# zgbkdlm/fbs

Hardware: AMD Instinct MI355X
Metric: particle-steps/sec (N x T per Gibbs sweep) (higher is better)
Workload: dtype f32; 1 GPU; 2-D Gaussian bridge toy (BASELINE config 2): N=65536 particles, T=500 steps, ts=linspace(0,2), analytic score, gibbs_kernel eb=True ef=False marg_y=False, conditional killing resampling; one step = one Gibbs sweep of a batch of 4 chain(s) (reference driver default nchains=4, vmapped); nparticles=65536, nsteps=500, nchains=4, du=1, dv=1, parallelism=1 GPU(s) x 4 independent chain(s) each, no collective

## Files before the change

### fbs_amd/csrc/fbsmi_lg.hip

```cpp
#include <hip/hip_runtime.h>

#include <array>
#include <cmath>
#include <cstdlib>
#include <map>
#include <mutex>
#include <new>
#include <string>
#include <utility>
#include <vector>

#include "../../include/fbsmi.h"
#include "fbsmi_device.h"
#include "fbsmi_em_path.h"
#include "fbsmi_host.h"

namespace fbsmi {

constexpr int kMaxNbSweep = 1024;
constexpr int kNumProfKernels = 3;

struct LgDev {
    int C;
    int Ctot, c0;
// ... 1379 lines not shown
    constexpr bool kPairNoise = DMAX <= 4;
    constexpr bool kEarlyRow = DMAX <= 2;
    const LgDev d = chain_view(dd, blockIdx.y);
    __shared__ TreeLds L;
    __shared__ float part[2][4 * HALVES];
    __shared__ int Jsh;
    __shared__ float lastsh;
    __shared__ float xish[kPairNoise ? DMAX : 1][NP];
    const int N = d.N, tid = threadIdx.x & (kBlock - 1), half = threadIdx.x / kBlock, lane = threadIdx.x & 63;
    const bool upper = half >= HP;
    const int pr = (int)threadIdx.x - (upper ? NP : 0);
    const int mL = blockIdx.x * NP + pr;
    const int m = upper ? mL + (N >> 1) : mL;
    const int tileb = m / kBlock;
    const uint32_t* kt = d.keytab + 8 * s;
    const uint32_t a0 = kt[0], a1 = kt[1], b0 = kt[2], b1 = kt[3], t0 = kt[6], t1 = kt[7];
    const int i_ref = d.bs[s], j_ref = d.bs[s + 1];
    const float* __restrict__ up = (s & 1) ? d.u1 : d.u0;
    float* __restrict__ un = (s & 1) ? d.u0 : d.u1;
    const float w_max = d.scal[1];
    const float inv_n = 1.0f / (float)N;
    TreeEntry te{};
    if (half == 0) te = tree_entry_loads(d, i_ref);
    float uref[DMAX];
#pragma unroll
    for (int r = 0; r < DMAX; ++r) uref[r] = r < d.du ? up[(size_t)r * N + i_ref] : 0.0f;
    const StepTables<DMAX> t = step_tables<DMAX>(d, s);
    const float* v_prev = d.vs + (size_t)s * d.dv;
    const float* v = d.vs + (size_t)(s + 1) * d.dv;
    const float* ustar = d.us_star + (size_t)(s + 1) * d.du;
    const float u3 = __uint_as_float(kt[4]);
    float xi[DMAX];
#pragma unroll
    for (int r = 0; r < DMAX; ++r) xi[r] = 0.0f;
    if (!kPairNoise) {
#pragma unroll
        for (int r = 0; r < DMAX; ++r)
            if (r < d.du) xi[r] = normal_at(t0, t1, (uint64_t)N * d.du, (uint64_t)m * d.du + r);
    } else if (upper) {
#pragma unroll
        for (int r = 0; r < DMAX; ++r) {
            if (r < d.du) {
                uint32_t lo_, hi_;
                random_bits_pair(t0, t1, (uint64_t)N * d.du, (uint64_t)mL * d.du + r, lo_, hi_);
                xish[r][pr] = normal_from_bits(lo_);
                xi[r] = normal_from_bits(hi_);
            }
        }
    }
    float last;
    int J;
    if (half == 0) {
        float rootW;
        J = tree_build(d, te, L, i_ref, u3, w_max, inv_n, last, rootW);
        if (tid == 0) {
            Jsh = J;
            lastsh = last;
        }
    } else {
#pragma unroll
        for (int k = 0; k < kTreeBuildBarriers; ++k) __syncthreads();
    }
    __syncthreads();
    J = Jsh;
    last = lastsh;
    int shift = (j_ref - J) % N;
    if (shift < 0) shift += N;
    int src = m - shift;
    if (src < 0) src += N;
    const float ws = d.w[src];
    float u[DMAX];
#pragma unroll
    for (int r = 0; r < DMAX; ++r) u[r] = r < d.du ? up[(size_t)r * N + src] : 0.0f;
    if (kPairNoise && !upper) {
#pragma unroll
        for (int r = 0; r < DMAX; ++r)
            if (r < d.du) xi[r] = xish[r][pr];
    }
    const float u1 = uniform_at(a0, a1, (uint64_t)N, (uint64_t)src);
    const float u2 = uniform_at(b0, b1, (uint64_t)N, (uint64_t)src);
    const float q = last * (1.0f - u2);
    float P = 0.0f, E = last;
    int tile, h, red = 0;
    tree_search_lds(L, d.nb, q, P, E, tile, h);
    const bool killed = u1 * w_max >= ws;
    float ucand[DMAX];
    if (killed) {
        const TreeRound rd = tree_round_load(d, tile, h);
        const int lo = tree_round_walk(rd, tile, h, q, P, E);
        const float4 w4 = *reinterpret_cast<const float4*>(d.w + lo);
        float4 ug[DMAX];
        float ue[DMAX];
        if (kEarlyRow) {
            const int en = lo + 4 < N ? lo + 4 : N - 1;
#pragma unroll
            for (int r = 0; r < DMAX; ++r) {
                ug[r] = r < d.du ? *reinterpret_cast<const float4*>(up + (size_t)r * N + lo) : make_float4(0.f, 0.f, 0.f, 0.f);
                ue[r] = r < d.du ? up[(size_t)r * N + en] : 0.0f;
            }
        }
        red = tree_leaves_walk(w4, lo, q, P, E);
        if (kEarlyRow) {
            const int k = red - lo;
#pragma unroll
            for (int r = 0; r < DMAX; ++r) {
                const float lo2 = (k & 1) ? ug[r].y : ug[r].x, hi2 = (k & 1) ? ug[r].w : ug[r].z;
                ucand[r] = k >= 4 ? ue[r] : ((k & 2) ? hi2 : lo2);
            }
        }
    }
    const bool pinned = m == j_ref;
    const int a = pinned ? i_ref : (killed ? red : src);
    if (killed && !pinned) {
#pragma unroll
        for (int r = 0; r < DMAX; ++r)
            if (r < d.du) u[r] = kEarlyRow ? ucand[r] : up[(size_t)r * N + a];
    }
    if (pinned) {
#pragma unroll
        for (int r = 0; r < DMAX; ++r) u[r] = uref[r];
    }
    if (d.As) d.As[(size_t)s * N + m] = a;
#pragma unroll
    for (int r = 0; r < DMAX; ++r) {
        if (r < d.du) {
            const float dr = drift_row<DMAX>(t, r, u, v_prev);
            float x = (u[r] + dr * t.dt) + t.sd * xi[r];
            if (pinned) x = ustar[r];
            un[(size_t)r * N + m] = x;
            if (d.uss) d.uss[((size_t)(s + 1) * N + m) * d.du + r] = x;
        }
    }
    const float l = lg_loglik<DMAX>(t, u, v, v_prev);
    d.lw[m] = l;
    float mx, sx;
    {
        const int wv = (threadIdx.x >> 6) & 3, h4 = half * 4;
        const float mw = wave_max(l);
        if (lane == 0) part[0][h4 + wv] = mw;
        __syncthreads();
        mx = fmaxf(fmaxf(part[0][h4], part[0][h4 + 1]), fmaxf(part[0][h4 + 2], part[0][h4 + 3]));
        TreePath pth;
        const float sw_ = wave_upsweep(fbsmi_expf(l - finite_or_zero_f(mx)), pth);
        if (lane == 0) part[1][h4 + wv] = sw_;
        __syncthreads();
        sx = (part[1][h4] + part[1][h4 + 1]) + (part[1][h4 + 2] + part[1][h4 + 3]);
    }
    if (tid == 0) {
        d.bmax[tileb] = mx;
        d.bsumexp[tileb] = sx;
    }
}

template <int DMAX>
__global__ void __launch_bounds__(kBlock) k_lg_prop2t(LgDev dd, int s) {
    const LgDev d = chain_view(dd, blockIdx.y);
    __shared__ TreeLds L;
    __shared__ float xch2[2][8];
    const int N = d.N, half = N >> 1, tid = threadIdx.x;
    const uint32_t* kt = d.keytab + 8 * s;
    const uint32_t a0 = kt[0], a1 = kt[1], b0 = kt[2], b1 = kt[3], t0 = kt[6], t1 = kt[7];
    const int i_ref = d.bs[s], j_ref = d.bs[s + 1];
    const int mA = blockIdx.x * kBlock + tid;
    const int m[2] = {mA, mA + half};
    const float* __restrict__ up = (s & 1) ? d.u1 : d.u0;
    float* __restrict__ un = (s & 1) ? d.u0 : d.u1;
    const float w_max = d.scal[1];
    const float inv_n = 1.0f / (float)N;
    const TreeEntry te = tree_entry_loads(d, i_ref);
    float uref[DMAX];
#pragma unroll
    for (int r = 0; r < DMAX; ++r) uref[r] = r < d.du ? up[(size_t)r * N + i_ref] : 0.0f;
    const StepTables<DMAX> t = step_tables<DMAX>(d, s);
    const float* v_prev = d.vs + (size_t)s * d.dv;
    const float* v = d.vs + (size_t)(s + 1) * d.dv;
    const float* ustar = d.us_star + (size_t)(s + 1) * d.du;
    const float u3 = __uint_as_float(kt[4]);
    float xi[2][DMAX];
#pragma unroll
    for (int r = 0; r < DMAX; ++r) {
        xi[0][r] = 0.0f;
        xi[1][r] = 0.0f;
        if (r < d.du) {
            uint32_t lo_, hi_;
            random_bits_pair(t0, t1, (uint64_t)N * d.du, (uint64_t)mA * d.du + r, lo_, hi_);
            xi[0][r] = normal_from_bits(lo_);
            xi[1][r] = normal_from_bits(hi_);
        }
    }
    float last;
    float rootW_unused;
    const int J = tree_build(d, te, L, i_ref, u3, w_max, inv_n, last, rootW_unused);
    int shift = (j_ref - J) % N;
    if (shift < 0) shift += N;
    int src[2];
    src[0] = mA - shift;
    if (src[0] < 0) src[0] += N;
    const bool a_low = src[0] < half;
    src[1] = a_low ? src[0] + half : src[0] - half;
    const int pbase = a_low ? src[0] : src[1];
    float ws[2], u[2][DMAX];
#pragma unroll
    for (int h2 = 0; h2 < 2; ++h2) {
        ws[h2] = d.w[src[h2]];
#pragma unroll
        for (int r = 0; r < DMAX; ++r) u[h2][r] = r < d.du ? up[(size_t)r * N + src[h2]] : 0.0f;
    }
    uint32_t k_lo, k_hi, r_lo, r_hi;
    random_bits_pair(a0, a1, (uint64_t)N, (uint64_t)pbase, k_lo, k_hi);
    random_bits_pair(b0, b1, (uint64_t)N, (uint64_t)pbase, r_lo, r_hi);
    const float u1[2] = {fbsmi_bits_to_unit(a_low ? k_lo : k_hi), fbsmi_bits_to_unit(a_low ? k_hi : k_lo)};
    const float u2[2] = {fbsmi_bits_to_unit(a_low ? r_lo : r_hi), fbsmi_bits_to_unit(a_low ? r_hi : r_lo)};
    const float qK[2] = {last * (1.0f - u2[0]), last * (1.0f - u2[1])};
    float P[2] = {0.0f, 0.0f}, E[2] = {last, last};
    int tile[2], h[2], hi[2] = {0, 0};
    {
        auto walk2x2 = [&](const float2* hp0, const float2* hp1, int& h0, int& h1) {
            const float2 a0 = hp0[h0], a1 = hp1[h1];
            const float4 c0 = *reinterpret_cast<const float4*>(hp0 + 2 * h0), c1 = *reinterpret_cast<const float4*>(hp1 + 2 * h1);
            const bool g0 = tree_walk(a0, qK[0], P[0], E[0]), g1 = tree_walk(a1, qK[1], P[1], E[1]);
            const bool k0 = tree_walk(g0 ? make_float2(c0.x, c0.y) : make_float2(c0.z, c0.w), qK[0], P[0], E[0]);
            const bool k1 = tree_walk(g1 ? make_float2(c1.x, c1.y) : make_float2(c1.z, c1.w), qK[1], P[1], E[1]);
            h0 = 4 * h0 + (g0 ? 0 : 2) + (k0 ? 0 : 1);
            h1 = 4 * h1 + (g1 ? 0 : 2) + (k1 ? 0 : 1);
        };
        auto walk1x2 = [&](const float2* hp0, const float2* hp1, int& h0, int& h1) {
            const float2 n0 = hp0[h0], n1 = hp1[h1];
            h0 = 2 * h0 + (tree_walk(n0, qK[0], P[0], E[0]) ? 0 : 1);
            h1 = 2 * h1 + (tree_walk(n1, qK[1], P[1], E[1]) ? 0 : 1);
        };
        const int nb = d.nb;
        int h0 = kBlock / nb, h1 = h0, lv = 31 - __builtin_clz(nb);
        for (; lv >= 2; lv -= 2) walk2x2(L.topW, L.topW, h0, h1);
        if (lv) walk1x2(L.topW, L.topW, h0, h1);
        tile[0] = h0 - kBlock;
        tile[1] = h1 - kBlock;
        const float2 *m0 = L.midW + tile[0] * kMidN, *m1 = L.midW + tile[1] * kMidN;
        h0 = h1 = 1;
        static_assert(kMidLv == 3 || kMidLv == 4, "walk of the tile levels kept in LDS");
        walk2x2(m0, m1, h0, h1);
        if (kMidLv == 4) walk2x2(m0, m1, h0, h1);
        else walk1x2(m0, m1, h0, h1);
        h[0] = h0;
        h[1] = h1;
    }
    const bool killed[2] = {u1[0] * w_max >= ws[0], u1[1] * w_max >= ws[1]};
    {
        TreeRound rd0{}, rd1{};
        if (killed[0]) rd0 = tree_round_load(d, tile[0], h[0]);
        if (killed[1]) rd1 = tree_round_load(d, tile[1], h[1]);
        int lo0 = 0, lo1 = 0;
        float4 w40 = make_float4(0.f, 0.f, 0.f, 0.f), w41 = w40;
        if (killed[0]) {
            lo0 = tree_round_walk(rd0, tile[0], h[0], qK[0], P[0], E[0]);
            w40 = *reinterpret_cast<const float4*>(d.w + lo0);
        }
        if (killed[1]) {
            lo1 = tree_round_walk(rd1, tile[1], h[1], qK[1], P[1], E[1]);
            w41 = *reinterpret_cast<const float4*>(d.w + lo1);
        }
        if (killed[0]) hi[0] = tree_leaves_walk(w40, lo0, qK[0], P[0], E[0]);
        if (killed[1]) hi[1] = tree_leaves_walk(w41, lo1, qK[1], P[1], E[1]);
    }
    float lnew[2];
#pragma unroll
    for (int h2 = 0; h2 < 2; ++h2) {
        const bool pinned = m[h2] == j_ref;
        const int a = pinned ? i_ref : (killed[h2] ? hi[h2] : src[h2]);
        if (killed[h2] && !pinned) {
#pragma unroll
            for (int r = 0; r < DMAX; ++r)
                if (r < d.du) u[h2][r] = up[(size_t)r * N + a];
        }
        if (pinned) {
#pragma unroll
            for (int r = 0; r < DMAX; ++r) u[h2][r] = uref[r];
        }
        if (d.As) d.As[(size_t)s * N + m[h2]] = a;
#pragma unroll
        for (int r = 0; r < DMAX; ++r) {
            if (r < d.du) {
                const float dr = drift_row<DMAX>(t, r, u[h2], v_prev);
                float x = (u[h2][r] + dr * t.dt) + t.sd * xi[h2][r];
                if (pinned) x = ustar[r];
                un[(size_t)r * N + m[h2]] = x;
                if (d.uss) d.uss[((size_t)(s + 1) * N + m[h2]) * d.du + r] = x;
            }
        }
        lnew[h2] = lg_loglik<DMAX>(t, u[h2], v, v_prev);
        d.lw[m[h2]] = lnew[h2];
    }
    float mxA, sxA, mxB, sxB;
    block_lse_partial2(lnew[0], lnew[1], xch2[0], xch2[1], mxA, sxA, mxB, sxB);
    if (tid == 0) {
        const int tb = blockIdx.x + (d.nb >> 1);
        d.bmax[blockIdx.x] = mxA;
        d.bsumexp[blockIdx.x] = sxA;
        d.bmax[tb] = mxB;
        d.bsumexp[tb] = sxB;
    }
}

template <int DMAX>
__global__ void __launch_bounds__(kBlock) k_lg_prop2(LgDev dd, int s) {
    const LgDev d = chain_view(dd, blockIdx.y);
    __shared__ float xch[2][8];
// ... 1582 lines not shown
    const float diff = prop_ell - old_ell;
    const float log_acc = (diff < 0.0f || diff != diff) ? diff : 0.0f;
    const float z = uniform_at(p.pk[4 * c + 2], p.pk[4 * c + 3], 1, 0);
    const bool acc = fbsmi_logf(z) < log_acc;
    __syncthreads();
    float* samples = (float*)p.out[0];
    float* uT = p.uT + (size_t)c * p.du;
    const float* new_uT = p.usT + ((size_t)c * p.N + p.which_u) * p.du;
    for (int r = threadIdx.x; r < p.du; r += kBlock) {
        const float x = acc ? new_uT[r] : uT[r];
        uT[r] = x;
        if (samples) samples[((size_t)it * p.C + c) * p.du + r] = x;
    }
    if (acc) {
        const size_t nys = ((size_t)p.T + 1) * p.dv;
        float* ys = p.ys + (size_t)c * nys;
        const float* prop = p.prop_ys + (size_t)c * nys;
        for (size_t e = threadIdx.x; e < nys; e += kBlock) ys[e] = prop[e];
    }
    if (threadIdx.x == 0) {
        if (acc) p.log_ell[c] = prop_ell;
        const size_t o = (size_t)it * p.C + c;
        if (p.out[1]) ((float*)p.out[1])[o] = fbsmi_expf(log_acc);
        if (p.out[2]) ((uint8_t*)p.out[2])[o] = acc ? 1 : 0;
        if (p.out[3]) ((float*)p.out[3])[o] = prop_ell;
        if (p.out[4]) ((float*)p.out[4])[o] = old_ell;
    }
}

constexpr int kFsBlockMax = 128;

__global__ void __launch_bounds__(kFsBlockMax) k_fs_front(PmDev p) {
    const int b = blockIdx.y;
    __shared__ uint32_t sk[2];
    __shared__ float syT[kFsBlockMax];
    if (threadIdx.x == 0) {
        const uint32_t k0 = p.ikeys[2 * b], k1 = p.ikeys[2 * b + 1];
        uint32_t f0, f1;
        split_at(k0, k1, 3, 0, sk[0], sk[1]);
        split_at(k0, k1, 3, 2, f0, f1);
        p.fkeys[2 * b] = f0;
        p.fkeys[2 * b + 1] = f1;
        split_at(f0, f1, 2, 0, p.pk[4 * b], p.pk[4 * b + 1]);
    }
    __syncthreads();
    const int T = p.T, dv = p.dv;
    const bool live = (int)threadIdx.x < dv;
    const int j = live ? (int)threadIdx.x : dv - 1;
    const uint32_t s0 = sk[0], s1 = sk[1];
    const uint64_t n = (uint64_t)T * dv;
    float* vs = p.vs + (size_t)b * ((size_t)T + 1) * dv;
    float r = p.y0[j];
    if (live) vs[(size_t)T * dv + j] = r;
    for (int k0 = 0; k0 < T; k0 += kPmChunk) {
        float f[kPmChunk], sq[kPmChunk], z[kPmChunk];
#pragma unroll
        for (int i = 0; i < kPmChunk; ++i) {
            const int k = k0 + i < T ? k0 + i : T - 1;
            f[i] = p.F[k];
            sq[i] = p.sqQ[k];
            z[i] = normal_at(s0, s1, n, (uint64_t)k * dv + j);
        }
#pragma unroll
        for (int i = 0; i < kPmChunk; ++i) {
            if (k0 + i < T) {
                r = f[i] * r + sq[i] * z[i];
                if (live) vs[(size_t)(T - 1 - k0 - i) * dv + j] = r;
            }
        }
    }
    if (live) syT[j] = r;
    __syncthreads();
    for (int u = threadIdx.x; u < p.du; u += blockDim.x) {
        double s = 0.0;
        for (int cc = 0; cc < dv; ++cc) s = s + p.gain[(size_t)u * dv + cc] * ((double)syT[cc] - p.m_v[cc]);
        p.mcond[(size_t)b * p.du + u] = (float)(p.m_u[u] + s);
    }
}

__global__ void __launch_bounds__(kFsBlockMax) k_fs_tail(PmDev p) {
    const int b = blockIdx.y;
    const float* row0 = p.usT + (size_t)b * p.N * p.du;
    for (int r = threadIdx.x; r < p.du; r += blockDim.x) p.uT[(size_t)b * p.du + r] = row0[r];
    if (threadIdx.x == 0) p.log_ell[b] = p.ell[b];
}

}

using namespace fbsmi;

__global__ void k_xcc_probe(int* out) {
    if (threadIdx.x == 0) {
        uint32_t id;
        asm volatile("s_getreg_b32 %0, hwreg(HW_REG_XCC_ID)" : "=s"(id));
        out[blockIdx.x] = (int)(id & 15);
    }
}

static bool xcd_round_robin_holds() {
    static const int ok = [] {
        if (const char* e = getenv("FBSMI_PIN_CHECK"))
            if (atoi(e) == 0) return 1;
        constexpr int kProbeBlocks = 64;
        int* dev = nullptr;
        int host[kProbeBlocks];
        if (hipMalloc(&dev, sizeof(host)) != hipSuccess) return 0;
        bool good = hipMemset(dev, 0xff, sizeof(host)) == hipSuccess;
        if (good) {
            k_xcc_probe<<<kProbeBlocks, 64, 0, nullptr>>>(dev);
            good = hipMemcpy(host, dev, sizeof(host), hipMemcpyDeviceToHost) == hipSuccess;
        }
        (void)hipFree(dev);
        if (!good) return 0;
        unsigned seen = 0;
        for (int b = 0; b < kProbeBlocks; ++b) {
            if (host[b] < 0 || host[b] > 15 || host[b] != host[b & 7]) return 0;
            if (b < 8) seen |= 1u << host[b];
        }
        return __builtin_popcount(seen) == 8 ? 1 : 0;
    }();
    return ok != 0;
}

constexpr int kStreamPool = 4;
static hipStream_t pool_stream(int g) {
    static std::mutex mu;
    static std::map<int, std::array<hipStream_t, kStreamPool>> pools;
    int dev = 0;
    (void)hipGetDevice(&dev);
    const int i = ((g % kStreamPool) + kStreamPool) % kStreamPool;
    std::lock_guard<std::mutex> lock(mu);
    hipStream_t& slot = pools[dev][i];
    if (!slot) {
        hipStream_t st = nullptr;
        if (hipStreamCreateWithFlags(&st, hipStreamNonBlocking) != hipSuccess) return nullptr;
        slot = st;
    }
    return slot;
}

struct fbsmi_lg_sweep {
    LgDev d{};
    int items = 1, dmax = 2;
    std::vector<void*> allocs;
    hipStream_t stream = nullptr;
    hipEvent_t ev_in = nullptr, ev_out = nullptr;
    hipGraphExec_t graph_single = nullptr;
    hipGraphExec_t graph_chain = nullptr;
    bool profile = false;
    int two_slot_prop = -1;
    bool tree_step = true;
    bool tree_plus1 = true;
    int tree_halves = -1;
    bool pin = true;
    bool wide_pin = true;
    bool em = false;
    EmDev emd{};
    bool bridge = false;
    BridgeDev brd{};
    std::vector<hipEvent_t> prof_ev[kNumProfKernels];
    double prof_us[kNumProfKernels] = {0, 0, 0};
    int64_t prof_n[kNumProfKernels] = {0, 0, 0};
};

namespace {

void read_switches(fbsmi_lg_sweep* s) {
    auto env = [](const char* name, int unset) {
        const char* e = getenv(name);
        return e ? atoi(e) : unset;
    };
    if (const char* e = getenv("FBSMI_TWO_SLOT_PROP")) s->two_slot_prop = atoi(e) != 0 ? 1 : 0;
    if (const char* e = getenv("FBSMI_TREE_HALVES")) s->tree_halves = atoi(e) == 1 ? 1 : (atoi(e) == 4 ? 4 : 2);
    s->tree_step = env("FBSMI_TREE_STEP", 1) != 0;
    s->tree_plus1 = env("FBSMI_TREE_PLUS1", 1) != 0;
    s->pin = env("FBSMI_PIN", 1) != 0;
    s->wide_pin = env("FBSMI_WIDE_PIN", 1) != 0;
}

template <typename T>
int dev_alloc(fbsmi_lg_sweep* s, T** p, size_t count) {
    void* q = nullptr;
    FBSMI_HIP_TRY(hipMalloc(&q, sizeof(T) * (count ? count : 1)));
    FBSMI_HIP_TRY(hipMemset(q, 0, sizeof(T) * (count ? count : 1)));
    s->allocs.push_back(q);
    *p = (T*)q;
    return 0;
}

struct Slab {
    std::vector<std::pair<void**, size_t>> reqs;
    size_t bytes = 0;

    template <typename T>
    void request(T** p, size_t count) {
        reqs.push_back({(void**)p, bytes});
        bytes += (sizeof(T) * (count ? count : 1) + 255) & ~(size_t)255;
    }

    hipError_t commit(void** base) {
        hipError_t e = hipMalloc(base, bytes ? bytes : 256);
        if (e == hipSuccess) e = hipMemset(*base, 0, bytes ? bytes : 256);
        if (e != hipSuccess) return e;
        for (auto& r : reqs) *r.first = (char*)*base + r.second;
        reqs.clear();
        return hipSuccess;
    }
};

#define LG_DMAX(s, ...)                                                       \
    do {                                                                      \
        if ((s)->dmax == 1) { constexpr int DMAX = 1; __VA_ARGS__; }          \
        else if ((s)->dmax == 2) { constexpr int DMAX = 2; __VA_ARGS__; }     \
        else if ((s)->dmax == 4) { constexpr int DMAX = 4; __VA_ARGS__; }     \
        else { constexpr int DMAX = 16; __VA_ARGS__; }                        \
    } while (0)
#define LG_ITEMS(s, ...)                                                      \
    do {                                                                      \
        if ((s)->items == 1) { constexpr int ITEMS = 1; __VA_ARGS__; }        \
        else if ((s)->items == 4) { constexpr int ITEMS = 4; __VA_ARGS__; }   \
        else { constexpr int ITEMS = 16; __VA_ARGS__; }                       \
    } while (0)

struct ProfScope {
    fbsmi_lg_sweep* s;
    int which;
    hipStream_t st;
    ProfScope(fbsmi_lg_sweep* s_, int which_, hipStream_t st_) : s(s_), which(which_), st(st_) { mark(); }
    ~ProfScope() { mark(); }
    void mark() {
        if (s->profile) {
            hipEvent_t e;
            hipEventCreate(&e);
            hipEventRecord(e, st);
            s->prof_ev[which].push_back(e);
        }
    }
};

int launch_status(const char* what) {
    hipError_t e = hipGetLastError();
    return e == hipSuccess ? FBSMI_OK : fail(FBSMI_ERR_HIP, std::string(what) + " launch: " + hipGetErrorString(e));
}

int grid_1d(int64_t n, int per_block, int cap) {
    const int64_t g = (n + per_block - 1) / per_block;
    return (int)(g < 1 ? 1 : (g > cap ? cap : g));
}

struct WideGeom {
    int nrt, Kp, S;
    size_t lds;
    int nst;
    int u_tiles;
    int v_tile0;
    explicit WideGeom(const LgDev& d)
        : nrt((d.D + kWideTile - 1) / kWideTile), Kp((d.D + 15) / 16 * 16), S(wide_plane_row(Kp)), lds(wide_lds_bytes(S)),
          nst((d.N + kWideTile - 1) / kWideTile), u_tiles((d.du + kWideTile - 1) / kWideTile), v_tile0(d.du / kWideTile) {}
    int v_tiles() const { return nrt - v_tile0; }
};


void sweep_prologue(fbsmi_lg_sweep* s, hipStream_t st, int chain, const WideGeom& w) {
    const LgDev& d = s->d;
    const dim3 gtile(d.nb, d.C);
    k_lg_keys<<<dim3(1, d.C), kBlock, 0, st>>>(d, chain);
    if (s->em) {
        k_lg_em_noise<<<dim3(grid_1d((int64_t)d.T * s->emd.t.nsub * d.D, 256, 1024), d.C), 256, 0, st>>>(d, s->emd);
        k_lg_em_path<<<dim3(1, d.C), (unsigned)((d.D + 63) / 64 * 64), 0, st>>>(d, s->emd, 0);
    } else {
        k_lg_noise<<<dim3(grid_1d((int64_t)d.T * d.D, 256, 1024), d.C), 256, 0, st>>>(d);
        if (s->bridge)
            k_lg_bridge_noise<<<dim3(grid_1d((int64_t)d.T * ((s->brd.nsub * d.dv + 1) / 2), kBlock, 1024), d.C), kBlock, 0, st>>>(d, s->brd);
        k_lg_path<<<dim3((d.D + 63) / 64, d.C), 64, 0, st>>>(d, 0);
        if (s->bridge) k_lg_bridge<<<dim3(1, d.C), (unsigned)((d.dv + 63) / 64 * 64), 0, st>>>(d, s->brd);
    }
    if (d.wide) {
        k_lgw_init<<<gtile, kBlock, 0, st>>>(d);
        if (d.ef) {
            k_lgw_gemm<3><<<dim3(w.nst * w.v_tiles(), d.C), kBlock, w.lds, st>>>(d, 0, w.v_tile0, w.v_tiles(), w.Kp, w.S, 2, 1);
            if (d.N > kBlock) k_lgw_lse<<<gtile, kBlock, 0, st>>>(d);
        }
    } else LG_ITEMS(s, LG_DMAX(s, k_lg_init<ITEMS, DMAX><<<gtile, kBlock, 0, st>>>(d)));
}

void sweep_one_tile_persistent(fbsmi_lg_sweep* s, hipStream_t st) {
    const LgDev& d = s->d;
    LG_DMAX(s, k_lg_sweep1<DMAX><<<dim3(1, d.C), kBlock, 0, st>>>(d));
}

void sweep_one_tile_stepwise(fbsmi_lg_sweep* s, hipStream_t st, const WideGeom& w) {
    const LgDev& d = s->d;
    const int gwide = w.nst * w.nrt;
    const bool pinned = d.wide && s->wide_pin && xcd_round_robin_holds() && d.C == 1 && gwide <= 32;
    const int extra = grid_1d((int64_t)d.N * d.du, 1024, 16);
    for (int k = 0; k < d.T; ++k) {
        ProfScope p(s, 2, st);
        if (pinned) k_lgw_gemm<1><<<dim3(gwide * 8, d.C), kBlock, w.lds, st>>>(d, k, 0, w.nrt, w.Kp, w.S, 3, 8 + ((2 * d.c0) & 7));
        else if (d.wide) k_lgw_gemm<1><<<dim3(gwide + extra, d.C), kBlock, w.lds, st>>>(d, k, 0, w.nrt, w.Kp, w.S, 3, 0);
        else LG_DMAX(s, k_lg_step1<DMAX><<<dim3(1, d.C), kBlock, 0, st>>>(d, k));
    }
}

void step_norm_cdf(fbsmi_lg_sweep* s, hipStream_t st, int k, bool tree, dim3 g, const LgDev& dk) {
    {
        ProfScope p(s, 0, st);
        if (tree) k_lg_norm<1, 0, true><<<dim3(g.x * (dk.pin ? 8 : 1), g.y), kBlock, 0, st>>>(dk, k);
        else LG_ITEMS(s, k_lg_norm<ITEMS, 0><<<g, kBlock, 0, st>>>(dk, k));
    }
    if (tree) return;
    ProfScope p(s, 1, st);
    LG_ITEMS(s, k_lg_cdf<ITEMS, 0><<<g, kBlock, 0, st>>>(dk, k));
}

void sweep_steps_wide(fbsmi_lg_sweep* s, hipStream_t st, const WideGeom& w) {
    const LgDev& d = s->d;
    const dim3 gtile(d.nb, d.C), gwide(w.nst * w.nrt, d.C);
    constexpr int64_t kFatMin = 700;
    const bool fat = (int64_t)gwide.x * d.C > kFatMin;
    const bool fat_rowsum = fat && (d.D & 3) == 0 && (d.du & 3) == 0;
    LgDev dz = d;
    dim3 gz = gtile;
    if (fat) {
        const int64_t third = (((int64_t)d.N * d.du + 1) / 2 + 2) / 3;
        dz.nz = grid_1d(third, kBlock, 1024);
        gz = dim3(gtile.x + dz.nz, gtile.y);
    }
    for (int k = 0; k < d.T; ++k) {
        step_norm_cdf(s, st, k, false, gz, dz);
        ProfScope p(s, 2, st);
        k_lgw_anc<<<gz, kBlock, 0, st>>>(dz, k);
        if (fat_rowsum) k_lgw_gemm_fat<true><<<dim3(w.nst, d.C), kBlock, w.lds, st>>>(d, k, w.nrt, w.Kp, w.S);
        else if (fat) k_lgw_gemm_fat<false><<<dim3(w.nst, d.C), kBlock, w.lds, st>>>(d, k, w.nrt, w.Kp, w.S);
        else k_lgw_gemm<0><<<gwide, kBlock, w.lds, st>>>(d, k, 0, w.nrt, w.Kp, w.S, 3, 0);
        if (fat_rowsum) k_lg_lwpart<<<gtile, kBlock, 0, st>>>(d);
        else k_lgw_lse<<<gtile, kBlock, 0, st>>>(d);
    }
}

void sweep_steps_narrow(fbsmi_lg_sweep* s, hipStream_t st) {
    const LgDev& d = s->d;
    const int nb = d.nb;
    const dim3 gtile(nb, d.C);
    const bool two_slot = s->items == 1 && d.N % (2 * kBlock) == 0 &&
                          (s->two_slot_prop == 1 || (s->two_slot_prop < 0 && (int64_t)nb * d.C >= 5 * 256));
    const bool tree = s->tree_step && d.trW;
    for (int k = 0; k < d.T; ++k) {
        step_norm_cdf(s, st, k, tree, gtile, d);
        ProfScope p(s, 2, st);
        if (tree && two_slot && !d.plus1) {
            LG_DMAX(s, k_lg_prop2t<DMAX><<<dim3(nb / 2, d.C), kBlock, 0, st>>>(d, k));
        } else if (tree && !d.plus1 && nb % 4 == 0 && s->tree_halves == 4) {
            LG_DMAX(s, k_lg_prop1tp<DMAX, 4><<<dim3(nb / 4, d.C), 4 * kBlock, 0, st>>>(d, k));
        } else if (tree && !d.plus1 && nb % 2 == 0 && (s->tree_halves == 2 || (s->tree_halves < 0 && (int64_t)nb * d.C >= 2 * 256))) {
            LG_DMAX(s, k_lg_prop1tp<DMAX, 2><<<dim3(nb / 2, d.C), 2 * kBlock, 0, st>>>(d, k));
        } else if (tree) {
            LG_DMAX(s, k_lg_prop1t<DMAX, 1><<<dim3(nb * (d.pin ? 8 : 1), d.C), kBlock, 0, st>>>(d, k));
        } else if (two_slot) {
            LG_DMAX(s, k_lg_prop2<DMAX><<<dim3(nb / 2, d.C), kBlock, 0, st>>>(d, k));
        } else if (s->items == 1) {
            LG_DMAX(s, k_lg_prop1<DMAX><<<gtile, kBlock, 0, st>>>(d, k));
        } else {
            k_lg_heaps<<<dim3(kHeapSizeW / kBlock, d.C), kBlock, 0, st>>>(d);
            LG_ITEMS(s, LG_DMAX(s, k_lg_propQ<ITEMS, DMAX><<<gtile, kBlock, 0, st>>>(d, k)));
        }
    }
}

void sweep_epilogue(fbsmi_lg_sweep* s, hipStream_t st, int chain) {
    const LgDev& d = s->d;
    const dim3 gone(1, d.C), gtile(d.nb, d.C);
    if (d.eb) {
        LG_ITEMS(s, k_lg_norm<ITEMS, 1><<<gtile, kBlock, 0, st>>>(d, d.T));
        LG_ITEMS(s, k_lg_cdf<ITEMS, 1><<<gtile, kBlock, 0, st>>>(d, d.T));
        k_lg_force_move<<<gone, 64, 0, st>>>(d);
        const int gpath = (d.D + 63) / 64;
        if (s->em) k_lg_em_path<<<dim3(1, d.C), (unsigned)((d.D + 63) / 64 * 64), 0, st>>>(d, s->emd, 1);
        else k_lg_path<<<dim3(gpath > (d.T + 64) / 64 ? gpath : (d.T + 64) / 64, d.C), 64, 0, st>>>(d, 1);
    } else {
        LG_ITEMS(s, k_lg_norm<ITEMS, 2><<<gtile, kBlock, 0, st>>>(d, d.T));
        LG_ITEMS(s, k_lg_cdf<ITEMS, 2><<<gtile, kBlock, 0, st>>>(d, d.T));
        k_lg_backscan<<<gone, 256, 0, st>>>(d);
    }
    k_lg_export<<<dim3(grid_1d((int64_t)d.N * d.du, 256, 2048), d.C), 256, 0, st>>>(d);
    if (chain) {
        k_lg_advance<<<gone, 256, 0, st>>>(d);
        k_lg_advance_key<<<1, 64, 0, st>>>(d);
    }
}

int enqueue_sweep(fbsmi_lg_sweep* s, hipStream_t st, int chain) {
    const LgDev& d = s->d;
    const WideGeom w(d);
    sweep_prologue(s, st, chain, w);
    if (d.N <= kBlock) {
        if (d.wide || s->profile) sweep_one_tile_stepwise(s, st, w);
        else sweep_one_tile_persistent(s, st);
        if (d.wide) k_lgw_lse<<<dim3(d.nb, d.C), kBlock, 0, st>>>(d);
        else k_lg_lwpart<<<dim3(d.nb, d.C), kBlock, 0, st>>>(d);
    } else if (d.wide) sweep_steps_wide(s, st, w);
    else sweep_steps_narrow(s, st);
    sweep_epilogue(s, st, chain);
    return launch_status("sweep");
}

int run_sweep(fbsmi_lg_sweep* s, int chain, int use_graph) {
    return launch_captured(chain ? s->graph_chain : s->graph_single, s->stream, use_graph && !s->profile,
                           [&] { return enqueue_sweep(s, s->stream, chain); });
}

int join_in(fbsmi_lg_sweep* s, hipStream_t ust) {
    FBSMI_HIP_TRY(hipEventRecord(s->ev_in, ust));
    FBSMI_HIP_TRY(hipStreamWaitEvent(s->stream, s->ev_in, 0));
    return FBSMI_OK;
}

int join_out(fbsmi_lg_sweep* s, hipStream_t ust) {
    FBSMI_HIP_TRY(hipEventRecord(s->ev_out, s->stream));
    FBSMI_HIP_TRY(hipStreamWaitEvent(ust, s->ev_out, 0));
    return FBSMI_OK;
}

int collect_profile(fbsmi_lg_sweep* s) {
    if (!s->profile) return FBSMI_OK;
    FBSMI_HIP_TRY(hipStreamSynchronize(s->stream));
    for (int w = 0; w < kNumProfKernels; ++w) {
        auto& v = s->prof_ev[w];
        for (size_t i = 0; i + 1 < v.size(); i += 2) {
            float ms = 0.f;
            if (hipEventElapsedTime(&ms, v[i], v[i + 1]) == hipSuccess) {
                s->prof_us[w] += (double)ms * 1000.0;
                s->prof_n[w] += 1;
            }
        }
        for (auto e : v) hipEventDestroy(e);
        v.clear();
    }
    return FBSMI_OK;
}

}

extern "C" {

int fbsmi_lg_sweep_create(const fbsmi_lg_model* m, int32_t nparticles, int explicit_backward, int explicit_final,
                          int store_path, int32_t nchains, fbsmi_lg_sweep** out) {
    if (!m || !out || nparticles < 1 || m->du < 1 || m->dv < 1 || m->T < 1 || nchains < 1 || nchains > 65535)
        return fail(FBSMI_ERR_ARG, "lg_sweep_create: bad arguments");
    if (!m->G || !m->g || !m->sd || !m->lognorm || !m->F || !m->sqQ)
        return fail(FBSMI_ERR_ARG, "lg_sweep_create: null model table");
    const int D = m->du + m->dv;
    const bool wide = m->du > 16 || m->dv > 16;
    if (wide && (m->du > 128 || m->dv > 128))
        return fail(FBSMI_ERR_UNSUPPORTED, "lg_sweep: du, dv > 128 are not supported by the fused sweep");

    if (wide && (explicit_final ? nparticles + 1 : nparticles) > 131072)
        return fail(FBSMI_ERR_UNSUPPORTED, "lg_sweep: du, dv > 16 with more than 131072 particles is not supported");
    if (!explicit_backward && !store_path)
        return fail(FBSMI_ERR_ARG, "lg_sweep_create: explicit_backward=0 needs store_path (As, uss)");
    fbsmi_lg_sweep* s = new (std::nothrow) fbsmi_lg_sweep();
    if (!s) return fail(FBSMI_ERR_ARG, "out of host memory");
    auto bail = [s](int code, const std::string& msg) {
        fbsmi_lg_sweep_destroy(s);
        return fail(code, msg);
    };
    LgDev& d = s->d;
    d.C = nchains;
    d.Ctot = nchains;
    d.c0 = 0;
    d.nparticles = nparticles;
    d.N = explicit_final ? nparticles + 1 : nparticles;
    d.du = m->du;
    d.dv = m->dv;
    d.D = D;
    d.T = m->T;
    d.eb = explicit_backward ? 1 : 0;
    d.ef = explicit_final ? 1 : 0;
    d.store = store_path ? 1 : 0;
    d.dt = m->dt;
    d.lw_init = (float)(-log((double)nparticles));
    d.G = m->G; d.g = m->g; d.sd = m->sd; d.lognorm = m->lognorm; d.F = m->F; d.sqQ = m->sqQ;
    d.levels = bisect_levels(d.N);
    d.wide = wide ? 1 : 0;
    read_switches(s);
    s->items = fbsmi_tile_items(d.N);
    const int maxd = m->du > m->dv ? m->du : m->dv;
    s->dmax = maxd <= 1 ? 1 : (maxd <= 2 ? 2 : (maxd <= 4 ? 4 : 16));
    const int tile = kBlock * s->items;
    d.nb = (d.N + tile - 1) / tile;
    if (d.nb > kMaxNbSweep) return bail(FBSMI_ERR_UNSUPPORTED, "lg_sweep: more than 4M particles per device not supported yet");
    if (store_path) {
        const double bytes = (((double)d.T * d.N * 4.0) + ((double)(d.T + 1) * d.N * (d.du + 1) * 4.0)) * nchains;
        if (bytes > 200e9) return bail(FBSMI_ERR_UNSUPPORTED, "lg_sweep: path storage (T,N,du) does not fit device memory");
    }
    const size_t N = d.N, T = d.T, C = nchains;
    Slab slab;
    slab.request(&d.key, 2);
    slab.request(&d.keys, 2 * C);
    slab.request(&d.x0, C * d.du);
    slab.request(&d.y0, d.dv);
    slab.request(&d.bs, C * (T + 1));
    slab.request(&d.keytab, C * 8 * T);
    slab.request(&d.misc, C * 16);
    slab.request(&d.xi1, C * T * D);
    slab.request(&d.xi2, C * T * D);
    slab.request(&d.path, 1);
    slab.request(&d.us_star, C * (T + 1) * d.du);
    slab.request(&d.vs, C * (T + 1) * d.dv);
// ... 720 lines not shown
```

Measured before the change: 19.09 billion particle-steps/s.

## Add half-wave particle mapping variant of tree propagate kernel

Adds k_lg_prop1th, a variant of the multi-half tree propagate kernel in which each 64-lane wave covers particles from both halves of the population, one half per 32-lane half-wave. The two threefry outputs are exchanged with permlane32_swap instead of LDS, and the per-tile max and sum-exp reductions use half-wave shuffles. For small state dimensions the noise pairs are generated by the non-builder threads into LDS while the builder threads build the tree. It is enabled by default for the 2- and 4-half paths, aiming to cut random-number work and improve overlap, at the cost of more complex indexing and extra LDS.

```diff
diff --git a/fbs_amd/csrc/fbsmi_lg.hip b/fbs_amd/csrc/fbsmi_lg.hip
--- a/fbs_amd/csrc/fbsmi_lg.hip
+++ b/fbs_amd/csrc/fbsmi_lg.hip
@@ -1555,6 +1555,199 @@
     }
 }
 
+__device__ __forceinline__ float halfwave_max(float m) {
+    m = fmaxf(m, tree_partner<1>(m));
+    m = fmaxf(m, tree_partner<2>(m));
+    m = fmaxf(m, tree_partner<4>(m));
+    m = fmaxf(m, tree_partner<8>(m));
+    m = fmaxf(m, tree_partner<16>(m));
+    return m;
+}
+
+__device__ __forceinline__ float halfwave_sum(float s) {
+    const int lane = threadIdx.x & 63;
+#define FBSMI_HALFWAVE_LEVEL(m, M)                      \
+    {                                                   \
+        const float o_ = tree_partner<M>(s);            \
+        s = ((lane >> m) & 1) ? o_ + s : s + o_;        \
+    }
+    FBSMI_HALFWAVE_LEVEL(0, 1)
+    FBSMI_HALFWAVE_LEVEL(1, 2)
+    FBSMI_HALFWAVE_LEVEL(2, 4)
+    FBSMI_HALFWAVE_LEVEL(3, 8)
+    FBSMI_HALFWAVE_LEVEL(4, 16)
+#undef FBSMI_HALFWAVE_LEVEL
+    return s;
+}
+
+template <int DMAX, int HALVES>
+__global__ void __launch_bounds__(kBlock * HALVES) k_lg_prop1th(LgDev dd, int s) {
+    static_assert(HALVES == 2 || HALVES == 4, "two sides of HALVES / 2 tiles");
+    constexpr int HP = HALVES / 2, NP = kBlock * HP;
+    constexpr bool kPairNoise = DMAX <= 4;
+    constexpr bool kEarlyRow = DMAX <= 2;
+    const LgDev d = chain_view(dd, blockIdx.y);
+    __shared__ TreeLds L;
+    __shared__ __attribute__((aligned(16))) float part[2][2][HP][8];
+    __shared__ int Jsh;
+    __shared__ float lastsh;
+    __shared__ float xish[kPairNoise ? DMAX : 1][2 * NP];
+    const int N = d.N, hN = N >> 1, tid = threadIdx.x, lane = threadIdx.x & 63, wv = threadIdx.x >> 6;
+    const int hw = lane >> 5;
+    const bool builder = tid < kBlock;
+    const int pr = wv * 32 + (lane & 31);
+    const int mL = blockIdx.x * NP + pr;
+    const int m = mL + (hw ? hN : 0);
+    const int ts = wv >> 3, bk = wv & 7;
+    const int tileb = blockIdx.x * HP + ts + (hw ? d.nb >> 1 : 0);
+    const uint32_t* kt = d.keytab + 8 * s;
+    const uint32_t a0 = kt[0], a1 = kt[1], b0 = kt[2], b1 = kt[3], t0 = kt[6], t1 = kt[7];
+    const int i_ref = d.bs[s], j_ref = d.bs[s + 1];
+    const float* __restrict__ up = (s & 1) ? d.u1 : d.u0;
+    float* __restrict__ un = (s & 1) ? d.u0 : d.u1;
+    const float w_max = d.scal[1];
+    const float inv_n = 1.0f / (float)N;
+    TreeEntry te{};
+    if (builder) te = tree_entry_loads(d, i_ref);
+    float uref[DMAX];
+#pragma unroll
+    for (int r = 0; r < DMAX; ++r) uref[r] = r < d.du ? up[(size_t)r * N + i_ref] : 0.0f;
+    const StepTables<DMAX> t = step_tables<DMAX>(d, s);
+    const float* v_prev = d.vs + (size_t)s * d.dv;
+    const float* v = d.vs + (size_t)(s + 1) * d.dv;
+    const float* ustar = d.us_star + (size_t)(s + 1) * d.du;
+    const float u3 = __uint_as_float(kt[4]);
+    float xi[DMAX];
+#pragma unroll
+    for (int r = 0; r < DMAX; ++r) xi[r] = 0.0f;
+    if (!kPairNoise) {
+#pragma unroll
+        for (int r = 0; r < DMAX; ++r)
+            if (r < d.du) xi[r] = normal_at(t0, t1, (uint64_t)N * d.du, (uint64_t)m * d.du + r);
+    } else if (tid >= NP) {
+        const int p = tid - NP, own = (p >> 5) * 64 + (p & 31);
+        const int mp = blockIdx.x * NP + p;
+#pragma unroll
+        for (int r = 0; r < DMAX; ++r) {
+            if (r < d.du) {
+                uint32_t lo_, hi_;
+                random_bits_pair(t0, t1, (uint64_t)N * d.du, (uint64_t)mp * d.du + r, lo_, hi_);
+                xish[r][own] = normal_from_bits(lo_);
+                xish[r][own + 32] = normal_from_bits(hi_);
+            }
+        }
+    }
+    float last;
+    int J;
+    if (builder) {
+        float rootW;
+        J = tree_build(d, te, L, i_ref, u3, w_max, inv_n, last, rootW);
+        if (tid == 0) {
+            Jsh = J;
+            lastsh = last;
+        }
+    } else {
+#pragma unroll
+        for (int k = 0; k < kTreeBuildBarriers; ++k) __syncthreads();
+    }
+    __syncthreads();
+    J = Jsh;
+    last = lastsh;
+    int shift = (j_ref - J) % N;
+    if (shift < 0) shift += N;
+    int src = m - shift;
+    if (src < 0) src += N;
+    const float ws = d.w[src];
+    float u[DMAX];
+#pragma unroll
+    for (int r = 0; r < DMAX; ++r) u[r] = r < d.du ? up[(size_t)r * N + src] : 0.0f;
+    if (kPairNoise) {
+#pragma unroll
+        for (int r = 0; r < DMAX; ++r)
+            if (r < d.du) xi[r] = xish[r][tid];
+    }
+    const int c = src & (hN - 1);
+    const bool swp = (src >= hN) != (hw != 0);
+    uint32_t o0, o1;
+    threefry2x32(hw ? b0 : a0, hw ? b1 : a1, (uint32_t)c, (uint32_t)(c + hN), o0, o1);
+    const auto xw = __builtin_amdgcn_permlane32_swap(swp ? o1 : o0, swp ? o0 : o1, false, false);
+    const float u1 = fbsmi_bits_to_unit(xw[0]);
+    const float u2 = fbsmi_bits_to_unit(xw[1]);
+    const float q = last * (1.0f - u2);
+    float P = 0.0f, E = last;
+    int tile, h, red = 0;
+    tree_search_lds(L, d.nb, q, P, E, tile, h);
+    const bool killed = u1 * w_max >= ws;
+    float ucand[DMAX];
+    if (killed) {
+        const TreeRound rd = tree_round_load(d, tile, h);
+        const int lo = tree_round_walk(rd, tile, h, q, P, E);
+        const float4 w4 = *reinterpret_cast<const float4*>(d.w + lo);
+        float4 ug[DMAX];
+        float ue[DMAX];
+        if (kEarlyRow) {
+            const int en = lo + 4 < N ? lo + 4 : N - 1;
+#pragma unroll
+            for (int r = 0; r < DMAX; ++r) {
+                ug[r] = r < d.du ? *reinterpret_cast<const float4*>(up + (size_t)r * N + lo) : make_float4(0.f, 0.f, 0.f, 0.f);
+                ue[r] = r < d.du ? up[(size_t)r * N + en] : 0.0f;
+            }
+        }
+        red = tree_leaves_walk(w4, lo, q, P, E);
+        if (kEarlyRow) {
+            const int k = red - lo;
+#pragma unroll
+            for (int r = 0; r < DMAX; ++r) {
+                const float lo2 = (k & 1) ? ug[r].y : ug[r].x, hi2 = (k & 1) ? ug[r].w : ug[r].z;
+                ucand[r] = k >= 4 ? ue[r] : ((k & 2) ? hi2 : lo2);
+            }
+        }
+    }
+    const bool pinned = m == j_ref;
+    const int a = pinned ? i_ref : (killed ? red : src);
+    if (killed && !pinned) {
+#pragma unroll
+        for (int r = 0; r < DMAX; ++r)
+            if (r < d.du) u[r] = kEarlyRow ? ucand[r] : up[(size_t)r * N + a];
+    }
+    if (pinned) {
+#pragma unroll
+        for (int r = 0; r < DMAX; ++r) u[r] = uref[r];
+    }
+    if (d.As) d.As[(size_t)s * N + m] = a;
+#pragma unroll
+    for (int r = 0; r < DMAX; ++r) {
+        if (r < d.du) {
+            const float dr = drift_row<DMAX>(t, r, u, v_prev);
+            float x = (u[r] + dr * t.dt) + t.sd * xi[r];
+            if (pinned) x = ustar[r];
+            un[(size_t)r * N + m] = x;
+            if (d.uss) d.uss[((size_t)(s + 1) * N + m) * d.du + r] = x;
+        }
+    }
+    const float l = lg_loglik<DMAX>(t, u, v, v_prev);
+    d.lw[m] = l;
+    float mx, sx;
+    {
+        const float mw = halfwave_max(l);
+        if ((lane & 31) == 0) part[0][hw][ts][bk] = mw;
+        __syncthreads();
+        const float4 ma = *reinterpret_cast<const float4*>(&part[0][hw][ts][0]);
+        const float4 mb = *reinterpret_cast<const float4*>(&part[0][hw][ts][4]);
+        mx = fmaxf(fmaxf(fmaxf(ma.x, ma.y), fmaxf(ma.z, ma.w)), fmaxf(fmaxf(mb.x, mb.y), fmaxf(mb.z, mb.w)));
+        const float sw_ = halfwave_sum(fbsmi_expf(l - finite_or_zero_f(mx)));
+        if ((lane & 31) == 0) part[1][hw][ts][bk] = sw_;
+        __syncthreads();
+        const float4 sa = *reinterpret_cast<const float4*>(&part[1][hw][ts][0]);
+        const float4 sb = *reinterpret_cast<const float4*>(&part[1][hw][ts][4]);
+        sx = ((sa.x + sa.y) + (sa.z + sa.w)) + ((sb.x + sb.y) + (sb.z + sb.w));
+    }
+    if (bk == 0 && (lane & 31) == 0) {
+        d.bmax[tileb] = mx;
+        d.bsumexp[tileb] = sx;
+    }
+}
+
 template <int DMAX>
 __global__ void __launch_bounds__(kBlock) k_lg_prop2t(LgDev dd, int s) {
     const LgDev d = chain_view(dd, blockIdx.y);
@@ -3443,6 +3636,7 @@
     bool tree_step = true;
     bool tree_plus1 = true;
     int tree_halves = -1;
+    bool halfwave = true;
     bool pin = true;
     bool wide_pin = true;
     bool em = false;
@@ -3465,6 +3659,7 @@
     if (const char* e = getenv("FBSMI_TREE_HALVES")) s->tree_halves = atoi(e) == 1 ? 1 : (atoi(e) == 4 ? 4 : 2);
     s->tree_step = env("FBSMI_TREE_STEP", 1) != 0;
     s->tree_plus1 = env("FBSMI_TREE_PLUS1", 1) != 0;
+    s->halfwave = env("FBSMI_PROP_HALFWAVE", 1) != 0;
     s->pin = env("FBSMI_PIN", 1) != 0;
     s->wide_pin = env("FBSMI_WIDE_PIN", 1) != 0;
 }
@@ -3642,9 +3837,11 @@
         if (tree && two_slot && !d.plus1) {
             LG_DMAX(s, k_lg_prop2t<DMAX><<<dim3(nb / 2, d.C), kBlock, 0, st>>>(d, k));
         } else if (tree && !d.plus1 && nb % 4 == 0 && s->tree_halves == 4) {
-            LG_DMAX(s, k_lg_prop1tp<DMAX, 4><<<dim3(nb / 4, d.C), 4 * kBlock, 0, st>>>(d, k));
+            if (s->halfwave) LG_DMAX(s, k_lg_prop1th<DMAX, 4><<<dim3(nb / 4, d.C), 4 * kBlock, 0, st>>>(d, k));
+            else LG_DMAX(s, k_lg_prop1tp<DMAX, 4><<<dim3(nb / 4, d.C), 4 * kBlock, 0, st>>>(d, k));
         } else if (tree && !d.plus1 && nb % 2 == 0 && (s->tree_halves == 2 || (s->tree_halves < 0 && (int64_t)nb * d.C >= 2 * 256))) {
-            LG_DMAX(s, k_lg_prop1tp<DMAX, 2><<<dim3(nb / 2, d.C), 2 * kBlock, 0, st>>>(d, k));
+            if (s->halfwave) LG_DMAX(s, k_lg_prop1th<DMAX, 2><<<dim3(nb / 2, d.C), 2 * kBlock, 0, st>>>(d, k));
+            else LG_DMAX(s, k_lg_prop1tp<DMAX, 2><<<dim3(nb / 2, d.C), 2 * kBlock, 0, st>>>(d, k));
         } else if (tree) {
             LG_DMAX(s, k_lg_prop1t<DMAX, 1><<<dim3(nb * (d.pin ? 8 : 1), d.C), kBlock, 0, st>>>(d, k));
         } else if (two_slot) {
```

Measured after the change: 19.37 billion particle-steps/s, median of 6. 1.5% higher.
